# LudoMichaud/hlsjs-p2p-wrapper

Measured on AMD Instinct MI355X. Metric: segments/sec + P2P offload ratio, 1080p 6 Mb/s HLS at 1/2/4/8 MI355X, higher is better.
Workload: dtype uint8

## Files before the change

### hlsjs_p2p_wrapper_amd/ops/csrc/kernels/aes_cbc.hip

```cpp
#include "common.h"

#include "aes_dev.h"
#include "launch.h"

namespace hlsp2p {
namespace dev {

constexpr int kAesThreads = kAesImageThreads;
constexpr int kAesWgPerCu = 1;
constexpr int kBlk = 4;

typedef int v4i __attribute__((ext_vector_type(4)));
typedef unsigned int v4u __attribute__((ext_vector_type(4)));
constexpr uint32_t kOutOfRange = 0x80000000u;
typedef int v8i __attribute__((ext_vector_type(8)));
typedef float v16f __attribute__((ext_vector_type(16)));

struct AesCrc {
  const int64_t* mask_off;
  const v4i* wfrag;
  uint32_t* masks;
};
constexpr int kCrcSteps = crc::kFusedAesSteps;
static_assert(kCrcSteps == 8 && crc::kFusedMaskDwords == 64 && 64 * kBlk * 16 == crc::kChunkBytes,
              "a decrypt chunk is one CRC chunk: 64 lanes x kBlk blocks, one mask dword per lane");

__device__ __forceinline__ void crc_chunk_masks(const uint4 (&c)[kBlk], const v4i (&w)[kCrcSteps], int lane,
                                                uint32_t* __restrict__ out) {
  const v16f init = {8388608.f, 8388608.f, 8388608.f, 8388608.f, 8388608.f, 8388608.f, 8388608.f, 8388608.f,
                     8388608.f, 8388608.f, 8388608.f, 8388608.f, 8388608.f, 8388608.f, 8388608.f, 8388608.f};
  uint32_t m = 0;
  v16f acc = init;
#pragma unroll
  for (int j = 0; j < kBlk; ++j) {
    const uint32_t dw[4] = {c[j].x, c[j].y, c[j].z, c[j].w};
#pragma unroll
    for (int d = 0; d < 4; ++d) {
      const uint32_t x = dw[d];
      const v8i a = {static_cast<int>(x & 0x11111111u), static_cast<int>(x & 0x22222222u),
                     static_cast<int>(x & 0x44444444u), static_cast<int>((x >> 1) & 0x44444444u), 0, 0, 0, 0};
      const v4i& wv = w[4 * (j & 1) + d];
      const v8i b = {wv.x, wv.y, wv.z, wv.w, 0, 0, 0, 0};
      acc = __builtin_amdgcn_mfma_scale_f32_32x32x64_f8f6f4(a, b, acc, 4, 4, 0, 0, 0, 0);
    }
    if (j & 1) {
#pragma unroll
      for (int i = 0; i < 16; ++i) m = __builtin_amdgcn_alignbit(__float_as_uint(acc[i]), m, 1);
      acc = init;
    }
  }
  out[lane] = m;
}

struct AesHdr {
  const int64_t* off;
  uint4* rec;
};
constexpr uint32_t kDiv188Magic = 2924233053u;
static_assert(ts::kPacket == 188, "the header-record division");

template <int kCrc, int kHdr>
__global__ __launch_bounds__(kAesThreads, 1) void aes128_cbc_decrypt_kernel(
    const uint8_t* __restrict__ src, uint8_t* __restrict__ dst, const int64_t* __restrict__ src_off,
    const int64_t* __restrict__ dst_off, const int64_t* __restrict__ blk_prefix,
    const int64_t* __restrict__ chunk_prefix, const uint32_t* __restrict__ drk, const uint32_t* __restrict__ ivw,
    const uint32_t* __restrict__ tdl_g, const uint8_t* __restrict__ isb_g, int64_t* __restrict__ out_len, int nseg,
    int64_t total_chunks, int64_t per_wg, AesCrc crc, AesHdr hdr) {
  __shared__ uint32_t s_tab[kTdDwords + kIsDwords];
  const int tid = threadIdx.x;
  aes_image_fill(s_tab, tdl_g, isb_g, tid);
  __syncthreads();
  const uint8_t* s_bytes = reinterpret_cast<const uint8_t*>(s_tab);
  uint32_t td_base[4], is_base;
  aes_image_bases(tid, td_base, is_base);
  const int lane = tid & 63;
  constexpr int kWaves = kAesThreads / 64;

  const int64_t begin = static_cast<int64_t>(blockIdx.x) * per_wg;
  const int64_t end = begin + per_wg < total_chunks ? begin + per_wg : total_chunks;
  int cur = -1;
  uint32_t rk[44];
  int64_t so = 0, dof = 0, cstart = 0, cend = 0, nblk = 0, maskb = -1, hdrb = 0;
  __amdgpu_buffer_rsrc_t s_rsrc = __builtin_amdgcn_make_buffer_rsrc(const_cast<uint8_t*>(src), 0, 0, 0x00020000);
  __amdgpu_buffer_rsrc_t d_rsrc = __builtin_amdgcn_make_buffer_rsrc(dst, 0, 0, 0x00020000);
  v4i crc_w[kCrcSteps];
  if constexpr (kCrc == 1) {
#pragma unroll
    for (int d = 0; d < kCrcSteps; ++d) crc_w[d] = crc.wfrag[d * 64 + lane];
  }
  for (int64_t ch = uniform64(begin + (tid >> 6)); ch < end; ch += kWaves) {
    if (cur < 0 || ch >= cend) {
      cur = cur < 0 ? find_seg_wave(chunk_prefix, nseg, ch)
                    : __builtin_amdgcn_readfirstlane(advance_seg(chunk_prefix, cur, ch));
#pragma unroll
      for (int k = 0; k < 44; ++k) rk[k] = drk[cur * 44 + k];
      so = src_off[cur];
      dof = dst_off[cur];
      cstart = chunk_prefix[cur];
      cend = chunk_prefix[cur + 1];
      nblk = blk_prefix[cur + 1] - blk_prefix[cur];
      maskb = crc.mask_off != nullptr ? crc.mask_off[cur] : -1;
      if constexpr (kHdr == 1) hdrb = hdr.off[cur];
      s_rsrc = __builtin_amdgcn_make_buffer_rsrc(const_cast<uint8_t*>(src + so), 0, static_cast<int>(nblk * 16),
                                                 0x00020000);
      d_rsrc = __builtin_amdgcn_make_buffer_rsrc(dst + dof, 0, static_cast<int>(nblk * 16), 0x00020000);
    }
    const int64_t b0 = (ch - cstart) * (64 * kBlk) + lane;
    uint4 c[kBlk], pv[kBlk];
    const uint32_t boff = static_cast<uint32_t>(b0) << 4;
#pragma unroll
    for (int j = 0; j < kBlk; ++j) {
      const v4u q = __builtin_amdgcn_raw_buffer_load_b128(s_rsrc, boff + 1024u * j, 0, 0);
      c[j] = make_uint4(q[0], q[1], q[2], q[3]);
    }
#pragma unroll
    for (int j = 0; j < kBlk; ++j) {
      const uint32_t o = boff + 1024u * j;
      const v4u q = __builtin_amdgcn_raw_buffer_load_b128(s_rsrc, j == 0 && o == 0 ? kOutOfRange : o - 16u, 0, 0);
      pv[j] = make_uint4(q[0], q[1], q[2], q[3]);
    }
    if (ch == cstart && lane == 0) pv[0] = reinterpret_cast<const uint4*>(ivw)[cur];
    if constexpr (kCrc == 1) {
      if (maskb >= 0)
        crc_chunk_masks(c, crc_w, lane, crc.masks + maskb + (ch - cstart) * 64);
    }
    uint32_t st[kBlk][4];
#pragma unroll
    for (int j = 0; j < kBlk; ++j) {
      st[j][0] = c[j].x ^ rk[0]; st[j][1] = c[j].y ^ rk[1]; st[j][2] = c[j].z ^ rk[2]; st[j][3] = c[j].w ^ rk[3];
    }
    AES_ROUNDS_PIPELINED(kBlk, st, rk)
#pragma unroll
    for (int j = 0; j < kBlk; ++j) {
      uint32_t o0, o1, o2, o3;
      AES_FINAL(st[j][0], st[j][1], st[j][2], st[j][3], o0, o1, o2, o3, rk + 40, pv[j])
      const uint4 p = make_uint4(o0, o1, o2, o3);
      const int64_t b = b0 + 64 * j;
      const v4u pw = {o0, o1, o2, o3};
      __builtin_amdgcn_raw_buffer_store_b128(pw, d_rsrc, static_cast<uint32_t>(b) << 4, 0, 0);
      if constexpr (kHdr == 1) {
        const uint32_t b16 = static_cast<uint32_t>(b) << 4;
        const uint32_t q = __umulhi(b16 + 187u, kDiv188Magic) >> 7;
        if (q * 188u - b16 < 16u && b < nblk) hdr.rec[hdrb + q] = p;
      }
      if (b == nblk - 1) out_len[cur] = pkcs7_len(p, nblk * 16);
    }
  }
}

int aes_chunk_blocks() { return 64 * kBlk; }

namespace {
void aes_grid(int64_t total_chunks, int num_cu, int64_t& grid, int64_t& per_wg) {
  constexpr int64_t kWaves = kAesThreads / 64;
  const int64_t max_wg = static_cast<int64_t>(num_cu) * kAesWgPerCu;
  grid = (total_chunks + kWaves * 2 - 1) / (kWaves * 2);
  if (grid > max_wg) grid = max_wg;
  if (grid < 1) grid = 1;
  per_wg = (total_chunks + grid - 1) / grid;
  grid = (total_chunks + per_wg - 1) / per_wg;
}
}

hipError_t launch_aes128_cbc_decrypt(const AesDecryptArgs& a) {
  if (a.total_chunks <= 0) return hipSuccess;
  int64_t grid, per_wg;
  aes_grid(a.total_chunks, a.num_cu, grid, per_wg);
  const AesCrc crc{a.crc.mask_off, reinterpret_cast<const v4i*>(a.crc.wfrag), a.crc.masks};
  const AesHdr hdr{a.hdr.off, reinterpret_cast<uint4*>(a.hdr.rec)};
#define AES_LAUNCH(M, H)                                                                                        \
  hipLaunchKernelGGL((aes128_cbc_decrypt_kernel<M, H>), dim3(static_cast<unsigned>(grid)), dim3(kAesThreads), 0, \
                     a.stream, a.src, a.dst, a.src_off, a.dst_off, a.blk_prefix, a.chunk_prefix, a.drk, a.iv,     \
                     a.td0, a.isb, a.out_len, a.nseg, a.total_chunks, per_wg, crc, hdr)
  const bool with_hdr = hdr.off != nullptr && hdr.rec != nullptr;
  if (crc.mask_off == nullptr) {
    if (with_hdr) AES_LAUNCH(0, 1); else AES_LAUNCH(0, 0);
  } else {
    if (with_hdr) AES_LAUNCH(1, 1); else AES_LAUNCH(1, 0);
  }
#undef AES_LAUNCH
  return hipGetLastError();
}

}
}
```

### hlsjs_p2p_wrapper_amd/ops/csrc/kernels/aes_dev.h

```cpp
#pragma once
#include <hip/hip_runtime.h>
#include <stdint.h>

namespace hlsp2p {
namespace dev {

constexpr int kAesImageThreads = 1024;
constexpr int kTdDwords = 2 * 256 * 64;
constexpr int kIsDwords = 256 * 32;
constexpr uint32_t kIsRegion = 0x20000u;

#define AES_SEL(k) (0x0c020000u | ((4u + (k)) << 8))
#define AES_LDS32(addr) (*reinterpret_cast<const uint32_t*>(s_bytes + (addr)))
#define AES_IS(w, k) AES_LDS32(((((w) >> (8 * (k))) & 0xffu) << 7) + is_base)

#define AES_XOR3(a, b, c) __builtin_amdgcn_bitop3_b32((a), (b), (c), 0x96)

#define AES_TDA(t, w, k) __builtin_amdgcn_perm((w), td_base[t], AES_SEL(k))
#define AES_ROUND_READS(v, s)                                                                                     \
  do {                                                                                                            \
    uint32_t a_[16];                                                                                              \
    a_[0] = AES_TDA(0, s[0], 0); a_[1] = AES_TDA(1, s[3], 1); a_[2] = AES_TDA(2, s[2], 2); a_[3] = AES_TDA(3, s[1], 3);     \
    a_[4] = AES_TDA(0, s[1], 0); a_[5] = AES_TDA(1, s[0], 1); a_[6] = AES_TDA(2, s[3], 2); a_[7] = AES_TDA(3, s[2], 3);     \
    a_[8] = AES_TDA(0, s[2], 0); a_[9] = AES_TDA(1, s[1], 1); a_[10] = AES_TDA(2, s[0], 2); a_[11] = AES_TDA(3, s[3], 3);   \
    a_[12] = AES_TDA(0, s[3], 0); a_[13] = AES_TDA(1, s[2], 1); a_[14] = AES_TDA(2, s[1], 2); a_[15] = AES_TDA(3, s[0], 3); \
    _Pragma("unroll") for (int q_ = 0; q_ < 16; ++q_) v[q_] = AES_LDS32(a_[q_]);                                  \
  } while (0)
#define AES_ROUND_XORS(s, v, k)                                                                                   \
  do {                                                                                                            \
    s[0] = AES_XOR3(AES_XOR3(v[0], v[1], v[2]), v[3], (k)[0]);                                                    \
    s[1] = AES_XOR3(AES_XOR3(v[4], v[5], v[6]), v[7], (k)[1]);                                                    \
    s[2] = AES_XOR3(AES_XOR3(v[8], v[9], v[10]), v[11], (k)[2]);                                                  \
    s[3] = AES_XOR3(AES_XOR3(v[12], v[13], v[14]), v[15], (k)[3]);                                                \
  } while (0)

#define AES_FINAL(s0, s1, s2, s3, o0, o1, o2, o3, k, px)                                                      \
  o0 = __builtin_amdgcn_bitop3_b32(__builtin_amdgcn_perm(AES_IS(s3, 1), AES_IS(s0, 0), 0x0c0c0500u),               \
                                   __builtin_amdgcn_perm(AES_IS(s1, 3), AES_IS(s2, 2), 0x07020c0cu), (k)[0], 0x96) ^ \
       (px).x;                                                                                                    \
  o1 = __builtin_amdgcn_bitop3_b32(__builtin_amdgcn_perm(AES_IS(s0, 1), AES_IS(s1, 0), 0x0c0c0500u),               \
                                   __builtin_amdgcn_perm(AES_IS(s2, 3), AES_IS(s3, 2), 0x07020c0cu), (k)[1], 0x96) ^ \
       (px).y;                                                                                                    \
  o2 = __builtin_amdgcn_bitop3_b32(__builtin_amdgcn_perm(AES_IS(s1, 1), AES_IS(s2, 0), 0x0c0c0500u),               \
                                   __builtin_amdgcn_perm(AES_IS(s3, 3), AES_IS(s0, 2), 0x07020c0cu), (k)[2], 0x96) ^ \
       (px).z;                                                                                                    \
  o3 = __builtin_amdgcn_bitop3_b32(__builtin_amdgcn_perm(AES_IS(s2, 1), AES_IS(s3, 0), 0x0c0c0500u),               \
                                   __builtin_amdgcn_perm(AES_IS(s0, 3), AES_IS(s1, 2), 0x07020c0cu), (k)[3], 0x96) ^ \
       (px).w;

#define AES_ROUNDS_PIPELINED(N, st, rk)                                                                           \
  _Pragma("unroll") for (int r_ = 1; r_ < 10; ++r_) {                                                             \
    const uint32_t* k_ = (rk) + 4 * r_;                                                                           \
    uint32_t v_[2][16];                                                                                           \
    AES_ROUND_READS(v_[0], st[0]);                                                                                \
    _Pragma("unroll") for (int j_ = 1; j_ < (N); ++j_) {                                                          \
      AES_ROUND_READS(v_[j_ & 1], st[j_]);                                                                        \
      AES_ROUND_XORS(st[j_ - 1], v_[(j_ - 1) & 1], k_);                                                           \
    }                                                                                                             \
    AES_ROUND_XORS(st[(N) - 1], v_[((N) - 1) & 1], k_);                                                           \
  }

__device__ __forceinline__ void aes_image_fill(uint32_t* s_tab, const uint32_t* __restrict__ tdl_g,
                                               const uint8_t* __restrict__ isb_g, int tid) {
  static_assert(kTdDwords == 32 * kAesImageThreads && kIsDwords == 8 * kAesImageThreads, "fill map");
  uint32_t td[16], is[8];
#pragma unroll
  for (int k = 0; k < 16; ++k) td[k] = tdl_g[(tid >> 6) + 16 * k];
#pragma unroll
  for (int k = 0; k < 8; ++k) is[k] = isb_g[(tid >> 5) + 32 * k];
  const int half = (tid >> 5) & 1;
#pragma unroll
  for (int k = 0; k < 32; ++k) {
    const uint32_t v = td[k & 15];
    const int rot = 8 * (2 * (k >> 4) + half);
    s_tab[tid + k * kAesImageThreads] = rot ? __builtin_amdgcn_alignbit(v, v, 32 - rot) : v;
  }
#pragma unroll
  for (int k = 0; k < 8; ++k) s_tab[kTdDwords + tid + k * kAesImageThreads] = is[k] * 0x01010101u;
}

__device__ __forceinline__ void aes_image_bases(int tid, uint32_t td_base[4], uint32_t& is_base) {
  const uint32_t l4 = static_cast<uint32_t>(tid & 31) << 2;
  td_base[0] = l4;
  td_base[1] = 128u | l4;
  td_base[2] = 0x10000u | l4;
  td_base[3] = 0x10000u | 128u | l4;
  is_base = kIsRegion + l4;
}

__device__ __forceinline__ int64_t pkcs7_len(uint4 p, int64_t nbytes) {
  const uint32_t pad = p.w >> 24;
  if (pad < 1 || pad > 16) return -1;
  const uint32_t w[4] = {p.x, p.y, p.z, p.w};
  bool ok = true;
#pragma unroll
  for (int b = 0; b < 16; ++b) {
    const uint32_t byte = (w[b >> 2] >> (8 * (b & 3))) & 0xff;
    if (b >= 16 - static_cast<int>(pad) && byte != pad) ok = false;
  }
  return ok ? nbytes - static_cast<int64_t>(pad) : -1;
}

__device__ __forceinline__ int64_t uniform64(int64_t v) {
  const uint32_t lo = __builtin_amdgcn_readfirstlane(static_cast<uint32_t>(v));
  const uint32_t hi = __builtin_amdgcn_readfirstlane(static_cast<uint32_t>(static_cast<uint64_t>(v) >> 32));
  return static_cast<int64_t>((static_cast<uint64_t>(hi) << 32) | lo);
}

}
}
```

Measured before the change: 18960.

## Prefetch next chunk's ciphertext during AES rounds and pipeline final round

In the non-CRC variant, the next chunk's ciphertext and previous-block loads are issued as buffer loads before and after the AES rounds, so memory latency overlaps with table-lookup compute. The final round is split into reads and combines and software-pipelined across blocks, the same way the middle rounds already are. Header-record stores now go through a bounds-checked buffer resource instead of a branch, and padding-length extraction moves to one lane after the loop. This adds register pressure from the double-buffered c/pv arrays and relies on an explicit waitcnt encoding.

```diff
diff --git a/hlsjs_p2p_wrapper_amd/ops/csrc/kernels/aes_cbc.hip b/hlsjs_p2p_wrapper_amd/ops/csrc/kernels/aes_cbc.hip
--- a/hlsjs_p2p_wrapper_amd/ops/csrc/kernels/aes_cbc.hip
+++ b/hlsjs_p2p_wrapper_amd/ops/csrc/kernels/aes_cbc.hip
@@ -25,7 +25,7 @@
 static_assert(kCrcSteps == 8 && crc::kFusedMaskDwords == 64 && 64 * kBlk * 16 == crc::kChunkBytes,
               "a decrypt chunk is one CRC chunk: 64 lanes x kBlk blocks, one mask dword per lane");
 
-__device__ __forceinline__ void crc_chunk_masks(const uint4 (&c)[kBlk], const v4i (&w)[kCrcSteps], int lane,
+__device__ __forceinline__ void crc_chunk_masks(const v4u (&c)[kBlk], const v4i (&w)[kCrcSteps], int lane,
                                                 uint32_t* __restrict__ out) {
   const v16f init = {8388608.f, 8388608.f, 8388608.f, 8388608.f, 8388608.f, 8388608.f, 8388608.f, 8388608.f,
                      8388608.f, 8388608.f, 8388608.f, 8388608.f, 8388608.f, 8388608.f, 8388608.f, 8388608.f};
@@ -80,46 +80,53 @@
   const int64_t end = begin + per_wg < total_chunks ? begin + per_wg : total_chunks;
   int cur = -1;
   uint32_t rk[44];
-  int64_t so = 0, dof = 0, cstart = 0, cend = 0, nblk = 0, maskb = -1, hdrb = 0;
+  int64_t cstart = 0, cend = 0, maskb = -1;
+  uint32_t nblk = 0;
   __amdgpu_buffer_rsrc_t s_rsrc = __builtin_amdgcn_make_buffer_rsrc(const_cast<uint8_t*>(src), 0, 0, 0x00020000);
   __amdgpu_buffer_rsrc_t d_rsrc = __builtin_amdgcn_make_buffer_rsrc(dst, 0, 0, 0x00020000);
+  __amdgpu_buffer_rsrc_t h_rsrc = __builtin_amdgcn_make_buffer_rsrc(dst, 0, 0, 0x00020000);
   v4i crc_w[kCrcSteps];
   if constexpr (kCrc == 1) {
 #pragma unroll
     for (int d = 0; d < kCrcSteps; ++d) crc_w[d] = crc.wfrag[d * 64 + lane];
   }
+  constexpr bool kPrefetch = kCrc == 0;
+  v4u c[kBlk], pv[kBlk];
   for (int64_t ch = uniform64(begin + (tid >> 6)); ch < end; ch += kWaves) {
-    if (cur < 0 || ch >= cend) {
+    const bool fresh = cur < 0 || ch >= cend;
+    if (fresh) {
       cur = cur < 0 ? find_seg_wave(chunk_prefix, nseg, ch)
                     : __builtin_amdgcn_readfirstlane(advance_seg(chunk_prefix, cur, ch));
 #pragma unroll
       for (int k = 0; k < 44; ++k) rk[k] = drk[cur * 44 + k];
-      so = src_off[cur];
-      dof = dst_off[cur];
       cstart = chunk_prefix[cur];
       cend = chunk_prefix[cur + 1];
-      nblk = blk_prefix[cur + 1] - blk_prefix[cur];
+      nblk = static_cast<uint32_t>(blk_prefix[cur + 1] - blk_prefix[cur]);
       maskb = crc.mask_off != nullptr ? crc.mask_off[cur] : -1;
-      if constexpr (kHdr == 1) hdrb = hdr.off[cur];
-      s_rsrc = __builtin_amdgcn_make_buffer_rsrc(const_cast<uint8_t*>(src + so), 0, static_cast<int>(nblk * 16),
-                                                 0x00020000);
-      d_rsrc = __builtin_amdgcn_make_buffer_rsrc(dst + dof, 0, static_cast<int>(nblk * 16), 0x00020000);
-    }
-    const int64_t b0 = (ch - cstart) * (64 * kBlk) + lane;
-    uint4 c[kBlk], pv[kBlk];
-    const uint32_t boff = static_cast<uint32_t>(b0) << 4;
-#pragma unroll
-    for (int j = 0; j < kBlk; ++j) {
-      const v4u q = __builtin_amdgcn_raw_buffer_load_b128(s_rsrc, boff + 1024u * j, 0, 0);
-      c[j] = make_uint4(q[0], q[1], q[2], q[3]);
-    }
-#pragma unroll
-    for (int j = 0; j < kBlk; ++j) {
-      const uint32_t o = boff + 1024u * j;
-      const v4u q = __builtin_amdgcn_raw_buffer_load_b128(s_rsrc, j == 0 && o == 0 ? kOutOfRange : o - 16u, 0, 0);
-      pv[j] = make_uint4(q[0], q[1], q[2], q[3]);
-    }
-    if (ch == cstart && lane == 0) pv[0] = reinterpret_cast<const uint4*>(ivw)[cur];
+      s_rsrc = __builtin_amdgcn_make_buffer_rsrc(const_cast<uint8_t*>(src + src_off[cur]), 0,
+                                                 static_cast<int>(nblk * 16u), 0x00020000);
+      d_rsrc = __builtin_amdgcn_make_buffer_rsrc(dst + dst_off[cur], 0, static_cast<int>(nblk * 16u), 0x00020000);
+      if constexpr (kHdr == 1) {
+        const uint32_t nrec = __umulhi(nblk * 16u + 187u, kDiv188Magic) >> 7;
+        h_rsrc = __builtin_amdgcn_make_buffer_rsrc(hdr.rec + uniform64(hdr.off[cur]), 0,
+                                                   static_cast<int>(nrec * 16u), 0x00020000);
+      }
+    }
+    const uint32_t cb = static_cast<uint32_t>(ch - cstart) * (64u * kBlk);
+    const uint32_t boff = (cb + lane) << 4;
+    if (!kPrefetch || fresh) {
+#pragma unroll
+      for (int j = 0; j < kBlk; ++j) c[j] = __builtin_amdgcn_raw_buffer_load_b128(s_rsrc, boff + 1024u * j, 0, 0);
+#pragma unroll
+      for (int j = 0; j < kBlk; ++j) {
+        const uint32_t o = boff + 1024u * j;
+        pv[j] = __builtin_amdgcn_raw_buffer_load_b128(s_rsrc, j == 0 && o == 0 ? kOutOfRange : o - 16u, 0, 0);
+      }
+      if (cb == 0 && lane == 0) pv[0] = reinterpret_cast<const v4u*>(ivw)[cur];
+      if constexpr (kPrefetch) {
+        __builtin_amdgcn_s_waitcnt(0x0f70);
+      }
+    }
     if constexpr (kCrc == 1) {
       if (maskb >= 0)
         crc_chunk_masks(c, crc_w, lane, crc.masks + maskb + (ch - cstart) * 64);
@@ -129,21 +136,44 @@
     for (int j = 0; j < kBlk; ++j) {
       st[j][0] = c[j].x ^ rk[0]; st[j][1] = c[j].y ^ rk[1]; st[j][2] = c[j].z ^ rk[2]; st[j][3] = c[j].w ^ rk[3];
     }
+    uint32_t noff = kOutOfRange, poff = kOutOfRange;
+    if constexpr (kPrefetch) {
+      const int64_t nch = ch + kWaves;
+      const bool same = nch < cend && nch < end;
+      noff = same ? boff + kWaves * (1024u * kBlk) : kOutOfRange;
+      poff = same ? noff - 16u : kOutOfRange;
+#pragma unroll
+      for (int j = 0; j < kBlk; ++j) c[j] = __builtin_amdgcn_raw_buffer_load_b128(s_rsrc, noff + 1024u * j, 0, 0);
+    }
     AES_ROUNDS_PIPELINED(kBlk, st, rk)
+    uint32_t o[kBlk][4];
+    AES_FINAL_PIPELINED(kBlk, st, o, rk + 40, pv);
+    if constexpr (kPrefetch) {
+#pragma unroll
+      for (int j = 0; j < kBlk; ++j) pv[j] = __builtin_amdgcn_raw_buffer_load_b128(s_rsrc, poff + 1024u * j, 0, 0);
+    }
 #pragma unroll
     for (int j = 0; j < kBlk; ++j) {
-      uint32_t o0, o1, o2, o3;
-      AES_FINAL(st[j][0], st[j][1], st[j][2], st[j][3], o0, o1, o2, o3, rk + 40, pv[j])
-      const uint4 p = make_uint4(o0, o1, o2, o3);
-      const int64_t b = b0 + 64 * j;
-      const v4u pw = {o0, o1, o2, o3};
-      __builtin_amdgcn_raw_buffer_store_b128(pw, d_rsrc, static_cast<uint32_t>(b) << 4, 0, 0);
-      if constexpr (kHdr == 1) {
-        const uint32_t b16 = static_cast<uint32_t>(b) << 4;
+      const v4u pw = {o[j][0], o[j][1], o[j][2], o[j][3]};
+      __builtin_amdgcn_raw_buffer_store_b128(pw, d_rsrc, boff + 1024u * j, 0, 0);
+    }
+    if constexpr (kHdr == 1) {
+#pragma unroll
+      for (int j = 0; j < kBlk; ++j) {
+        const uint32_t b16 = boff + 1024u * j;
         const uint32_t q = __umulhi(b16 + 187u, kDiv188Magic) >> 7;
-        if (q * 188u - b16 < 16u && b < nblk) hdr.rec[hdrb + q] = p;
-      }
-      if (b == nblk - 1) out_len[cur] = pkcs7_len(p, nblk * 16);
+        const v4u pw = {o[j][0], o[j][1], o[j][2], o[j][3]};
+        __builtin_amdgcn_raw_buffer_store_b128(pw, h_rsrc, q * 188u - b16 < 16u ? q << 4 : kOutOfRange, 0, 0);
+      }
+    }
+    if (ch == cend - 1) {
+      const uint32_t r = nblk - 1u - cb;
+      const int jl = static_cast<int>(r >> 6);
+      uint4 p = make_uint4(o[0][0], o[0][1], o[0][2], o[0][3]);
+#pragma unroll
+      for (int j = 1; j < kBlk; ++j)
+        if (jl == j) p = make_uint4(o[j][0], o[j][1], o[j][2], o[j][3]);
+      if (lane == static_cast<int>(r & 63u)) out_len[cur] = pkcs7_len(p, static_cast<int64_t>(nblk) * 16);
     }
   }
 }
diff --git a/hlsjs_p2p_wrapper_amd/ops/csrc/kernels/aes_dev.h b/hlsjs_p2p_wrapper_amd/ops/csrc/kernels/aes_dev.h
--- a/hlsjs_p2p_wrapper_amd/ops/csrc/kernels/aes_dev.h
+++ b/hlsjs_p2p_wrapper_amd/ops/csrc/kernels/aes_dev.h
@@ -34,19 +34,35 @@
     s[3] = AES_XOR3(AES_XOR3(v[12], v[13], v[14]), v[15], (k)[3]);                                                \
   } while (0)
 
-#define AES_FINAL(s0, s1, s2, s3, o0, o1, o2, o3, k, px)                                                      \
-  o0 = __builtin_amdgcn_bitop3_b32(__builtin_amdgcn_perm(AES_IS(s3, 1), AES_IS(s0, 0), 0x0c0c0500u),               \
-                                   __builtin_amdgcn_perm(AES_IS(s1, 3), AES_IS(s2, 2), 0x07020c0cu), (k)[0], 0x96) ^ \
-       (px).x;                                                                                                    \
-  o1 = __builtin_amdgcn_bitop3_b32(__builtin_amdgcn_perm(AES_IS(s0, 1), AES_IS(s1, 0), 0x0c0c0500u),               \
-                                   __builtin_amdgcn_perm(AES_IS(s2, 3), AES_IS(s3, 2), 0x07020c0cu), (k)[1], 0x96) ^ \
-       (px).y;                                                                                                    \
-  o2 = __builtin_amdgcn_bitop3_b32(__builtin_amdgcn_perm(AES_IS(s1, 1), AES_IS(s2, 0), 0x0c0c0500u),               \
-                                   __builtin_amdgcn_perm(AES_IS(s3, 3), AES_IS(s0, 2), 0x07020c0cu), (k)[2], 0x96) ^ \
-       (px).z;                                                                                                    \
-  o3 = __builtin_amdgcn_bitop3_b32(__builtin_amdgcn_perm(AES_IS(s2, 1), AES_IS(s3, 0), 0x0c0c0500u),               \
-                                   __builtin_amdgcn_perm(AES_IS(s0, 3), AES_IS(s1, 2), 0x07020c0cu), (k)[3], 0x96) ^ \
-       (px).w;
+#define AES_FINAL_READS(v, s)                                                                                     \
+  do {                                                                                                            \
+    v[0] = AES_IS(s[0], 0); v[1] = AES_IS(s[3], 1); v[2] = AES_IS(s[2], 2); v[3] = AES_IS(s[1], 3);               \
+    v[4] = AES_IS(s[1], 0); v[5] = AES_IS(s[0], 1); v[6] = AES_IS(s[3], 2); v[7] = AES_IS(s[2], 3);               \
+    v[8] = AES_IS(s[2], 0); v[9] = AES_IS(s[1], 1); v[10] = AES_IS(s[0], 2); v[11] = AES_IS(s[3], 3);             \
+    v[12] = AES_IS(s[3], 0); v[13] = AES_IS(s[2], 1); v[14] = AES_IS(s[1], 2); v[15] = AES_IS(s[0], 3);           \
+  } while (0)
+#define AES_FINAL_WORD(v, i, kw, pw)                                                                              \
+  (__builtin_amdgcn_bitop3_b32(__builtin_amdgcn_perm(v[4 * (i) + 1], v[4 * (i)], 0x0c0c0500u),                    \
+                               __builtin_amdgcn_perm(v[4 * (i) + 3], v[4 * (i) + 2], 0x07020c0cu), (kw), 0x96) ^  \
+   (pw))
+#define AES_FINAL_COMBINE(o, v, k, px)                                                                            \
+  do {                                                                                                            \
+    o[0] = AES_FINAL_WORD(v, 0, (k)[0], (px).x);                                                                  \
+    o[1] = AES_FINAL_WORD(v, 1, (k)[1], (px).y);                                                                  \
+    o[2] = AES_FINAL_WORD(v, 2, (k)[2], (px).z);                                                                  \
+    o[3] = AES_FINAL_WORD(v, 3, (k)[3], (px).w);                                                                  \
+  } while (0)
+
+#define AES_FINAL_PIPELINED(N, st, o, k, px)                                                                      \
+  do {                                                                                                            \
+    uint32_t f_[2][16];                                                                                           \
+    AES_FINAL_READS(f_[0], st[0]);                                                                                \
+    _Pragma("unroll") for (int j_ = 1; j_ < (N); ++j_) {                                                          \
+      AES_FINAL_READS(f_[j_ & 1], st[j_]);                                                                        \
+      AES_FINAL_COMBINE(o[j_ - 1], f_[(j_ - 1) & 1], k, px[j_ - 1]);                                              \
+    }                                                                                                             \
+    AES_FINAL_COMBINE(o[(N) - 1], f_[((N) - 1) & 1], k, px[(N) - 1]);                                             \
+  } while (0)
 
 #define AES_ROUNDS_PIPELINED(N, st, rk)                                                                           \
   _Pragma("unroll") for (int r_ = 1; r_ < 10; ++r_) {                                                             \
```

New measurement: 18910. No clear change (-0.3%).
